# shiwanghua/swh-trl

Measured on AMD Instinct MI355X. Metric: GRPO step samples/sec (rollout+update), Qwen2.5-0.5B at 1/2/4/8 MI355X, higher is better.
Workload: dtype bf16; 1 GPU; configs[1]: Qwen2.5-0.5B GRPO bf16, group_size=8, 256-tok completions; model=Qwen2.5-0.5B (random init), global_batch=64, prompts_per_gpu=8, prompt_len=128, completion_len=256, seq_len=384, micro_batch=16, grad_accum=4, parallelism=dp1, layers=24

## Files before the change

include/swh_trl_amd.h:

```cpp
#ifndef SWH_TRL_AMD_H
#define SWH_TRL_AMD_H

#include <stdint.h>

#ifdef __cplusplus
extern "C" {
#endif

#define SWH_OK 0
#define SWH_E_ARG (-1)
#define SWH_E_LAUNCH (-2)
#define SWH_E_DTYPE (-3)

#define SWH_F32 0
#define SWH_BF16 1
#define SWH_F16 2

const char *swh_version(void);
const char *swh_status_string(int status);

typedef struct swh_launch_policy {
    int64_t wide_kmin;
    int32_t wide_gemm;
    int32_t wide_smax;
    int32_t wide_cb;
    int32_t gemm_ms;
    int32_t gemm_cb;
    int32_t gemm_s;
    int32_t gemm_persist;
    int32_t gemm_wn;
    int32_t gemm_tile;
    int32_t gemm_nw;
    int32_t xstream;
    int32_t lm_ring14;
    int32_t filt_wgs;
    int32_t wide_waves;
    int32_t attn_pair;
} swh_launch_policy;
int swh_launch_policy_default(swh_launch_policy *out);
int swh_get_launch_policy(swh_launch_policy *out);
int swh_set_launch_policy(const swh_launch_policy *p);

#define SWH_LOGP_ROUND_SCALED 1
int swh_logp_entropy_fwd(const void *logits, int dtype, int64_t rows_outer, int64_t rows_inner,
                         int64_t stride_outer, int64_t stride_inner, int64_t V, const int64_t *ids,
                         float temperature, int flags, float *logp, float *entropy, float *lse,
                         void *stream);

int swh_logp_bwd(const void *logits, int dtype, int64_t rows_outer, int64_t rows_inner,
                 int64_t stride_outer, int64_t stride_inner, int64_t V, const int64_t *ids,
                 float temperature, int flags, const float *lse, const float *dlogp, void *dlogits,
                 int64_t dstride_outer, int64_t dstride_inner, void *stream);
int swh_log_softmax_gather_exact(const void *logits, int dtype, int64_t rows_outer, int64_t rows_inner,
                                 int64_t stride_outer, int64_t stride_inner, int64_t V, const int64_t *ids,
                                 void *out, void *stream);


typedef struct {
    float temperature;
    float top_p;
    float min_p;
    float repetition_penalty;
    int32_t top_k;
    int32_t greedy;
    int32_t min_new_tokens;
    int32_t pad_token_id;
    int32_t n_eos;
    int32_t eos_ids[4];
} swh_sample_params;
int64_t swh_sample_workspace_bytes(int64_t B, int64_t V);
int swh_sample_step(const void *logits, int dtype, int64_t B, int64_t V, int64_t ld,
                    const swh_sample_params *params, const uint64_t *rng, const int32_t *step,
                    int32_t *finished,
                    uint32_t *seen, int64_t *out_tokens, int64_t out_ld, int64_t *cur_tokens,
                    float *out_logp, float *scores_out, void *workspace, void *stream);
int swh_seen_init(const int64_t *ids, const int32_t *mask, int64_t B, int64_t L, int64_t V,
                  uint32_t *seen, void *stream);
int swh_step_advance(int32_t *step, void *stream);

int swh_completion_mask(const int64_t *completion_ids, int64_t B, int64_t C, const int32_t *eos_ids,
                        int32_t n_eos, int32_t mask_truncated, int32_t *mask, int32_t *lengths,
                        int32_t *has_eos, void *stream);

int swh_group_advantage(const float *rewards_per_func, const float *weights, int64_t N, int64_t F,
                        int64_t G, int32_t scale_rewards, float *advantages, float *rewards,
                        float *group_mean, float *group_std, int32_t *zero_std, void *stream);

#define SWH_LOSS_GRPO 0
#define SWH_LOSS_BNPO 1
#define SWH_LOSS_DR_GRPO 2
// ... 186 lines not shown
```

swh_trl_amd/_lib.py:

```python
from __future__ import annotations

import ctypes as C
import os
import threading

_HERE = os.path.dirname(os.path.abspath(__file__))
LIB_PATH = os.path.join(_HERE, "libswh_trl_amd.so")

c_i32, c_i64, c_f32, c_vp, c_u64 = C.c_int32, C.c_int64, C.c_float, C.c_void_p, C.c_uint64

SWH_F32, SWH_BF16, SWH_F16 = 0, 1, 2
SWH_LOGP_ROUND_SCALED = 1
LOSS_TYPES = {"grpo": 0, "bnpo": 1, "dr_grpo": 2}
IS_LEVELS = {"token": 0, "sequence": 1}


class AttnView(C.Structure):
    _fields_ = [("base", C.c_void_p * 2), ("sb", c_i64 * 2), ("sh", c_i64 * 2), ("sl", c_i64 * 2),
                ("div", c_i32 * 2)]


class SampleParams(C.Structure):
    _fields_ = [("temperature", c_f32), ("top_p", c_f32), ("min_p", c_f32), ("repetition_penalty", c_f32),
                ("top_k", c_i32), ("greedy", c_i32), ("min_new_tokens", c_i32), ("pad_token_id", c_i32),
                ("n_eos", c_i32), ("eos_ids", c_i32 * 4)]


class GRPOLossParams(C.Structure):
    _fields_ = [("beta", c_f32), ("epsilon_low", c_f32), ("epsilon_high", c_f32), ("delta", c_f32),
                ("loss_type", c_i32), ("is_level", c_i32), ("max_completion_length", c_i32),
                ("num_segments", c_i32)]


class LaunchPolicy(C.Structure):
    _fields_ = [("wide_kmin", c_i64), ("wide_gemm", c_i32), ("wide_smax", c_i32), ("wide_cb", c_i32),
                ("gemm_ms", c_i32), ("gemm_cb", c_i32), ("gemm_s", c_i32), ("gemm_persist", c_i32),
                ("gemm_wn", c_i32), ("gemm_tile", c_i32), ("gemm_nw", c_i32), ("xstream", c_i32),
                ("lm_ring14", c_i32), ("filt_wgs", c_i32), ("wide_waves", c_i32), ("attn_pair", c_i32)]


SIGNATURES = {
    "swh_version": (C.c_char_p, []),
    "swh_status_string": (C.c_char_p, [c_i32]),
    "swh_launch_policy_default": (c_i32, [C.POINTER(LaunchPolicy)]),
    "swh_get_launch_policy": (c_i32, [C.POINTER(LaunchPolicy)]),
    "swh_set_launch_policy": (c_i32, [C.POINTER(LaunchPolicy)]),
    "swh_logp_entropy_fwd": (c_i32, [c_vp, c_i32, c_i64, c_i64, c_i64, c_i64, c_i64, c_vp, c_f32, c_i32,
                                     c_vp, c_vp, c_vp, c_vp]),
    "swh_log_softmax_gather_exact": (c_i32, [c_vp, c_i32, c_i64, c_i64, c_i64, c_i64, c_i64, c_vp, c_vp, c_vp]),
    "swh_logp_bwd": (c_i32, [c_vp, c_i32, c_i64, c_i64, c_i64, c_i64, c_i64, c_vp, c_f32, c_i32, c_vp, c_vp,
                             c_vp, c_i64, c_i64, c_vp]),
    "swh_sample_workspace_bytes": (c_i64, [c_i64, c_i64]),
    "swh_sample_step": (c_i32, [c_vp, c_i32, c_i64, c_i64, c_i64, C.POINTER(SampleParams), c_vp, c_vp, c_vp,
                                c_vp, c_vp, c_i64, c_vp, c_vp, c_vp, c_vp, c_vp]),
    "swh_seen_init": (c_i32, [c_vp, c_vp, c_i64, c_i64, c_i64, c_vp, c_vp]),
    "swh_step_advance": (c_i32, [c_vp, c_vp]),
    "swh_completion_mask": (c_i32, [c_vp, c_i64, c_i64, c_vp, c_i32, c_i32, c_vp, c_vp, c_vp, c_vp]),
    "swh_group_advantage": (c_i32, [c_vp, c_vp, c_i64, c_i64, c_i64, c_i32, c_vp, c_vp, c_vp, c_vp, c_vp,
                                    c_vp]),
    "swh_grpo_loss_workspace_bytes": (c_i64, [c_i64]),
    "swh_grpo_loss_fwd_bwd": (c_i32, [c_vp, c_vp, c_vp, c_vp, c_vp, c_vp, c_vp, c_vp, c_vp, c_i64, c_i64,
                                      C.POINTER(GRPOLossParams), c_vp, c_vp, c_vp, c_vp, c_vp, c_vp]),
    "swh_masked_whiten_workspace_bytes": (c_i64, [c_i64]),
    "swh_masked_whiten": (c_i32, [c_vp, c_vp, c_i64, c_i32, c_vp, c_vp, c_vp, c_vp]),
    "swh_gae_scan": (c_i32, [c_vp, c_vp, c_i64, c_i64, c_f32, c_f32, c_vp, c_vp, c_vp]),
    "swh_ppo_loss_workspace_bytes": (c_i64, [c_i64]),
    "swh_ppo_loss_fwd_bwd": (c_i32, [c_vp, c_vp, c_vp, c_vp, c_vp, c_vp, c_vp, c_vp, c_i64, c_i64, c_f32,
                                     c_f32, c_f32, c_vp, c_vp, c_vp, c_vp, c_vp, c_vp]),
    "swh_ppo_truncate": (c_i32, [c_vp, c_i64, c_i64, c_i64, c_i64, c_vp, c_vp, c_vp]),
    "swh_ppo_rewards": (c_i32, [c_vp, c_vp, c_i64, c_i64, c_i64, c_f32, c_i32, c_f32, c_i32, c_vp, c_vp, c_vp, c_vp,
                                c_i32, c_vp, c_vp, c_vp, c_vp, c_vp, c_vp]),
    "swh_value_head_fwd": (c_i32, [c_vp, c_i32, c_i64, c_i64, c_i64, c_vp, c_vp, c_vp, c_vp]),
    "swh_sqnorm_partials": (c_i64, [c_i64]),
    "swh_grad_sqnorm": (c_i32, [c_vp, c_i32, c_i64, c_vp, c_vp]),
    "swh_finalize_clip": (c_i32, [c_vp, c_i64, c_f32, c_vp, c_vp]),
    "swh_adamw": (c_i32, [c_vp, c_vp, c_vp, c_vp, c_i32, c_vp, c_i32, c_i64, c_f32, c_f32, c_f32, c_f32, c_f32,
                          c_i64, c_vp, c_vp, c_i32, c_vp]),
    "swh_accumulate": (c_i32, [c_vp, c_vp, c_i32, c_i64, c_f32, c_vp]),
    "swh_dw_reduce": (c_i32, [c_vp, c_i32, c_i64, c_vp, c_i32, c_vp]),
    "swh_gemm_nt": (c_i32, [c_vp, c_vp, c_vp, c_vp, c_i64, c_i64, c_i64, c_i64, c_i64, c_i64, c_vp]),
    "swh_gemm_nt256": (c_i32, [c_vp, c_vp, c_vp, c_vp, c_i64, c_i64, c_i64, c_i64, c_i64, c_i64, c_vp]),
    "swh_gemm_tn_partials": (c_i32, [c_vp, c_vp, c_vp, c_vp, c_i64, c_i64, c_i64, c_i64, c_i64, c_i32, c_vp]),
    "swh_gemm_tn256_partials": (c_i32, [c_vp, c_vp, c_vp, c_i64, c_i64, c_i64, c_i64, c_i64, c_i32, c_vp]),
    "swh_gemm_tn_fold": (c_i32, [c_vp, c_i32, c_i64, c_vp, c_i32, c_vp]),
    "swh_ema_mix": (c_i32, [c_vp, c_vp, c_i32, c_i64, c_f32, c_f32, c_vp]),
    "swh_rmsnorm_fwd": (c_i32, [c_vp, c_vp, c_vp, c_vp, c_i64, c_i64, c_f32, c_vp, c_vp, c_i32, c_vp]),
    "swh_rmsnorm_bwd": (c_i32, [c_vp, c_vp, c_vp, c_vp, c_i64, c_i64, c_vp, c_vp, c_i64, c_vp, c_i32, c_vp]),
    "swh_rmsnorm_dw_accum": (c_i32, [c_vp, c_i64, c_i64, c_vp, c_i32, c_vp]),
    "swh_colsum_partials": (c_i32, [c_vp, c_i64, c_i64, c_i64, c_vp, c_i32, c_vp]),
    "swh_layernorm_fwd": (c_i32, [c_vp, c_vp, c_vp, c_vp, c_i64, c_i64, c_f32, c_vp, c_vp, c_vp, c_vp, c_i32, c_vp]),
    "swh_layernorm_bwd_partial_rows": (c_i64, [c_i64, c_i64]),
# ... 153 lines not shown
```

swh_trl_amd/csrc/decode.hip:

```cpp
#include <cstdio>
#include <cstdlib>
#include <type_traits>

#include "common.hpp"

namespace swh {
int wide_gemm(const void *x, const void *w, int64_t M, int64_t N, int64_t K, float eps, const float *ss_in,
              const void *bias, void *residual, int32_t silu, void *y, int64_t ldy, float *ss_out, void *workspace,
              int64_t workspace_bytes, int64_t counter_bytes, int32_t packed, hipStream_t stream);
int64_t wide_gemm_slab_bytes(int64_t M, int64_t N, int64_t K, int32_t silu);
bool wide_gemm_eligible(int64_t M, int64_t N, int64_t K, int32_t silu);
int wide_pack(const void *src, const void *norm_w, int64_t N, int64_t K, int32_t silu, void *dst, hipStream_t stream);
int wide_lm_sample(const void *x, const void *w, int64_t M, int64_t V, int64_t K, float eps, const float *ss_in,
                   const swh_sample_params &p, const uint64_t *rng, const int32_t *step, LmPart *part, int *pstride,
                   hipStream_t stream);
int frag_pack(const void *src, const void *norm_w, int64_t N, int64_t K, int32_t silu, void *dst, hipStream_t stream);

namespace {

typedef __bf16 bf16x8 __attribute__((ext_vector_type(8)));
typedef float f32x4 __attribute__((ext_vector_type(4)));

constexpr int kRows = 64;
constexpr int64_t kCounterBytes = 1 << 16;

enum : int { EPI_PLAIN = 0, EPI_RESIDUAL = 1, EPI_SILU = 2 };

#ifdef SWH_GEMM_TRACE_ON
__device__ unsigned long long *g_gemm_trace;
#define SWH_GEMM_TRACE(i)                                                                                      \
    if (threadIdx.x == 0 && g_gemm_trace)                                                                      \
    g_gemm_trace[((int64_t)(blockIdx.z * gridDim.y + blockIdx.y) * gridDim.x + blockIdx.x) * 8 + (i)] =        \
        wall_clock64()
#else
#define SWH_GEMM_TRACE(i)
#endif

__device__ __forceinline__ void lds_barrier() { asm volatile("s_waitcnt lgkmcnt(0)\n\ts_barrier" ::: "memory"); }

__device__ __forceinline__ bf16x8 as_bf16x8(const uint4 &v) { return __builtin_bit_cast(bf16x8, v); }

typedef float f32x2 __attribute__((ext_vector_type(2)));
typedef __bf16 bf16x2 __attribute__((ext_vector_type(2)));
__device__ __forceinline__ uint32_t norm_pair(uint32_t xv, f32x2 w, float rs) {
    const f32x2 xf = {__uint_as_float(xv << 16), __uint_as_float(xv & 0xffff0000u)};
    const uint32_t tb = __builtin_bit_cast(uint32_t, __builtin_convertvector(xf * rs, bf16x2));
    const f32x2 tf = {__uint_as_float(tb << 16), __uint_as_float(tb & 0xffff0000u)};
    return __builtin_bit_cast(uint32_t, __builtin_convertvector(tf * w, bf16x2));
}
__device__ __forceinline__ uint4 norm_frag(const uint4 &xv, const float4 &w0, const float4 &w1, float rs) {
    return uint4{norm_pair(xv.x, f32x2{w0.x, w0.y}, rs), norm_pair(xv.y, f32x2{w0.z, w0.w}, rs),
                 norm_pair(xv.z, f32x2{w1.x, w1.y}, rs), norm_pair(xv.w, f32x2{w1.z, w1.w}, rs)};
}

__device__ __forceinline__ uint4 pack8(const float *v) {
    uint32_t o[4];
#pragma unroll
    for (int k = 0; k < 4; ++k)
        o[k] = (uint32_t)f32_to_bf16_bits(v[2 * k]) | ((uint32_t)f32_to_bf16_bits(v[2 * k + 1]) << 16);
    return uint4{o[0], o[1], o[2], o[3]};
}


struct GemmLds {
    int64_t nw_off, ss_off, body_off, xs_bytes, slots_off, total;
};
__host__ __device__ inline GemmLds gemm_lds(int cb, int mr, int nw, int krmax, int K, int nm, bool persist,
                                            int wn = 1) {
    GemmLds L;
    L.nw_off = 512;
    L.ss_off = L.nw_off + (nm == 1 ? (int64_t)krmax * 4 : 0);
    L.body_off = L.ss_off + (nm ? ((int64_t)mr * (K / 64) * 4 + 15) / 16 * 16 : 0);
    L.xs_bytes = (int64_t)mr * (krmax * 2 + 16);
    const int wk = nw / wn;
    const int64_t slots = (int64_t)(wk + 1) * 16 * cb * (mr + 4) * 4;
    L.slots_off = L.body_off + (persist ? L.xs_bytes : 0);
    int64_t end = L.body_off + L.xs_bytes;
    if (L.slots_off + slots > end) end = L.slots_off + slots;
    L.total = end;
    return L;
}


#ifndef SWH_KU
#define SWH_KU 4
#endif
#ifndef SWH_ROUND_PREFETCH
#define SWH_ROUND_PREFETCH 0
#endif
#ifndef SWH_W_NT
#define SWH_W_NT 0
#endif
__device__ __forceinline__ uint4 ld_w(const uint16_t *p) {
// ... 558 lines not shown
                    float b[8];
                    unpack16<SWH_BF16>(pre_ep, b);
#pragma unroll
                    for (int cc = 0; cc < 8; ++cc) v[cc] += b[cc];
                }
                *reinterpret_cast<uint4 *>(y + (int64_t)gr * ldy + gc) = pack8(v);
            }
        }
    }
    if constexpr (EPI == EPI_RESIDUAL) {
        if (ss_out) {
            __syncthreads();
            if (tid < MR && m0 + tid < M) {
                float ss = 0.f;
#pragma unroll
                for (int cc = 0; cc < 16; ++cc) ss = fmaf(slot(F, tid, cc), slot(F, tid, cc), ss);
                ss_out[(int64_t)(m0 + tid) * (N / 16) + n0 / 16] = ss;
            }
        }
    }
    SWH_GEMM_TRACE(6);
}

constexpr int kLmMaxKS = 32;

struct LmSample {
    swh_sample_params p;
    const uint64_t *rng;
    const int32_t *step;
    LmPart *part;
    int pstride;
    int fw = 0;
    int yf = 0;
    float2 *lpart = nullptr;
};

template <int CTRL>
__device__ __forceinline__ float dpp_f(float v) {
    return __builtin_bit_cast(float, __builtin_amdgcn_update_dpp(0, __builtin_bit_cast(int, v), CTRL, 0xF, 0xF, false));
}
__device__ __forceinline__ float row16_max(float v) {
    v = fmaxf(v, dpp_f<0xB1>(v));
    v = fmaxf(v, dpp_f<0x4E>(v));
    v = fmaxf(v, dpp_f<0x141>(v));
    return fmaxf(v, dpp_f<0x140>(v));
}
__device__ __forceinline__ float row16_sum(float v) {
    v += dpp_f<0xB1>(v);
    v += dpp_f<0x4E>(v);
    v += dpp_f<0x141>(v);
    return v + dpp_f<0x140>(v);
}

template <int NM, int EPI, bool BIAS, int SAMPLE, int KSC, int RD = 0>
__global__ __launch_bounds__(RD ? 768 : 512) void lm_head_kernel(const uint16_t *__restrict__ x, const uint16_t *__restrict__ w,
                                                      int M, int N, int K, const uint16_t *__restrict__ norm_w,
                                                      float eps, const float *__restrict__ ss_in,
                                                      const uint16_t *__restrict__ bias, uint16_t *__restrict__ y,
                                                      int ldy, LmSample smp) {
    extern __shared__ __attribute__((aligned(16))) unsigned char lds[];
    const int tid = threadIdx.x, lane = tid & 63, wid = tid >> 6, NT = blockDim.x, NW = NT >> 6;
    const int rl = lane & 15, kq = (lane >> 4) * 8, g = lane >> 4;
    const int nmt = (M + 63) / 64, mt = blockIdx.x % nmt, m0 = mt * 64;
    const int wgs = gridDim.x / nmt, wg = blockIdx.x / nmt;
    constexpr int KSA = KSC ? KSC : kLmMaxKS;
    const int ntile = (EPI == EPI_SILU) ? N / 8 : N / 16, KS = KSC ? KSC : K / 32, RS = K * 2 + 16;
    const GemmLds L = gemm_lds(1, 64, NW, K, K, NM, false);
    float *rstd_s = reinterpret_cast<float *>(lds);
    float *nw_s = reinterpret_cast<float *>(lds + L.nw_off);
    float *ssp = reinterpret_cast<float *>(lds + L.ss_off);
    unsigned char *xs = lds + L.body_off;
    const int tstep = wgs * NW;
    int t = wg + wgs * wid;
    SWH_GEMM_TRACE(0);

    static_assert(RD == 0 || (KSC != 0 && KSC % RD == 0 && 2 * RD == KSC), "RD: half of a compile-time tile");
    constexpr int KR = RD ? RD : KSA;
    uint4 bv[KR];
    auto wrow_of = [&](int tile) -> int64_t {
        if constexpr (EPI == EPI_SILU) return (rl < 8) ? tile * 8 + rl : N + tile * 8 + rl - 8;
        return (int64_t)tile * 16 + rl;
    };
    const int64_t wst = smp.fw ? 512 : 32;
    auto wbase = [&](int tile) -> const uint16_t * {
        return smp.fw ? w + ((int64_t)tile * KS * 64 + lane) * 8 : w + wrow_of(tile) * K + kq;
    };
    auto issue = [&](int tile) {
        const uint16_t *wr = wbase(tile);
#pragma unroll
        for (int ks = 0; ks < KR; ++ks)
            if (KSC || ks < KS) bv[ks] = ld_wt<EPI == EPI_SILU>(wr + ks * wst);
    };
    if (t < ntile) issue(t);
    const int nc = K / 64;
    const bool reg_rstd = NM == 2 && ss_in && 64 * 8 <= NT && nc <= 64;
    const bool use_ss = NM && ss_in && 64 * nc <= 4 * NT && !reg_rstd;
    float4 ssv[4];
    float4 ss8[8];
    uint4 nwv[2];
    if (reg_rstd) {
        const int r = min(m0 + (tid >> 3), M - 1), sub = tid & 7;
        const float4 *row = reinterpret_cast<const float4 *>(ss_in + (int64_t)r * (K / 16));
#pragma unroll
        for (int j = 0; j < 8; ++j)
            if (sub + 8 * j < nc) ss8[j] = row[sub + 8 * j];
    }
    if constexpr (NM != 0) {
        if (use_ss) {
#pragma unroll
            for (int q = 0; q < 4; ++q) {
                const int idx = min(tid + q * NT, 64 * nc - 1);
                const int r = idx / nc, c = idx - r * nc;
                ssv[q] = reinterpret_cast<const float4 *>(ss_in + (int64_t)min(m0 + r, M - 1) * (K / 16))[c];
            }
        }
        if constexpr (NM == 1) {
#pragma unroll
            for (int q = 0; q < 2; ++q) nwv[q] = reinterpret_cast<const uint4 *>(norm_w)[min(tid + q * NT, K / 8 - 1)];
        }
    }
    const int ppr = K / 8, jpl = (ppr + 63) >> 6;
    for (int r = wid; r < 64; r += NW) {
        const uint16_t *src = x + (int64_t)min(m0 + r, M - 1) * K;
        for (int j = 0; j < jpl; ++j) {
            const int c = lane + 64 * j;
            if (c < ppr)
                __builtin_amdgcn_global_load_lds(src + c * 8,
                                                 (__attribute__((address_space(3))) void *)(xs + r * RS + j * 1024),
                                                 16, 0, 0);
        }
    }
    if constexpr (NM != 0) {
        if (use_ss) {
#pragma unroll
            for (int q = 0; q < 4; ++q) {
                const int idx = tid + q * NT;
                if (idx < 64 * nc) ssp[idx] = ((ssv[q].x + ssv[q].y) + ssv[q].z) + ssv[q].w;
            }
        }
#pragma unroll
        for (int q = 0; q < 2; ++q)
            if (NM == 1 && tid + q * NT < K / 8) {
                float f[8];
                unpack16<SWH_BF16>(nwv[q], f);
                reinterpret_cast<float4 *>(nw_s)[2 * (tid + q * NT)] = float4{f[0], f[1], f[2], f[3]};
                reinterpret_cast<float4 *>(nw_s)[2 * (tid + q * NT) + 1] = float4{f[4], f[5], f[6], f[7]};
            }
    }
    SWH_GEMM_TRACE(1);
    asm volatile("s_waitcnt vmcnt(0)" ::: "memory");
    if (reg_rstd) {
        const int r = tid >> 3, sub = tid & 7;
        float v = 0.f;
#pragma unroll
        for (int j = 0; j < 8; ++j)
            if (sub + 8 * j < nc) v += ((ss8[j].x + ss8[j].y) + ss8[j].z) + ss8[j].w;
        v += __shfl_xor(v, 1);
        v += __shfl_xor(v, 2);
        v += __shfl_xor(v, 4);
        if (r < 64 && sub == 0) rstd_s[r] = rsqrtf(v / (float)K + eps);
    }
    lds_barrier();
    SWH_GEMM_TRACE(2);
    if (NM != 0 && !reg_rstd) {
        if (tid < 64) {
            float ssum = 0.f;
            if (use_ss) {
                for (int c = 0; c < nc; ++c) ssum += ssp[tid * nc + c];
            } else {
                for (int c = 0; c < ppr; ++c) {
                    float a[8];
                    unpack16<SWH_BF16>(*reinterpret_cast<const uint4 *>(xs + tid * RS + c * 16), a);
#pragma unroll
                    for (int k = 0; k < 8; ++k) ssum = fmaf(a[k], a[k], ssum);
                }
            }
            rstd_s[tid] = rsqrtf(ssum / (float)K + eps);
        }
        lds_barrier();
    }
    SWH_GEMM_TRACE(3);
    float rsr[4][4];
#pragma unroll
    for (int i = 0; i < 4; ++i)
#pragma unroll
        for (int e = 0; e < 4; ++e) rsr[i][e] = (NM == 2) ? rstd_s[i * 16 + 4 * g + e] : 1.f;
    if constexpr (NM == 1) {
        int r = tid / ppr, c = tid - r * ppr;
        const int rstep = NT / ppr, cstep = NT - rstep * ppr;
        while (r < 64) {
            uint4 *pv = reinterpret_cast<uint4 *>(xs + r * RS + c * 16);
            const float4 *wv = reinterpret_cast<const float4 *>(nw_s) + 2 * c;
            *pv = norm_frag(*pv, wv[0], wv[1], rstd_s[r]);
            r += rstep;
            c += cstep;
            if (c >= ppr) {
                c -= ppr;
                ++r;
            }
        }
        lds_barrier();
    }
    constexpr bool TDIV = SAMPLE == 2 || SAMPLE == 4, LOGP = SAMPLE >= 3;
    float bk[4][4];
    int32_t bi[4][4];
    uint32_t k0 = 0, k1 = 0, clo = 0, chi = 0;
    bool suppress = false;
    float temp = 1.f;
    float lm_run = kNegInf, ls_run = 0.f;
    if constexpr (SAMPLE) {
#pragma unroll
        for (int i = 0; i < 4; ++i)
#pragma unroll
            for (int e = 0; e < 4; ++e) {
                bk[i][e] = kNegInf;
                bi[i][e] = 0x7fffffff;
            }
        const int32_t step = *smp.step;
        const uint64_t seed = smp.rng[0], ctr = smp.rng[1] + (uint64_t)step;
        k0 = (uint32_t)seed;
        k1 = (uint32_t)(seed >> 32);
        clo = (uint32_t)ctr;
        chi = (uint32_t)(ctr >> 32);
        suppress = step < smp.p.min_new_tokens;
        temp = (!smp.p.greedy && smp.p.temperature != 1.0f) ? smp.p.temperature : 1.f;
    }
    for (; t < ntile; t += tstep) {
        f32x4 acc[4];
#pragma unroll
        for (int i = 0; i < 4; ++i) acc[i] = f32x4{0.f, 0.f, 0.f, 0.f};
        const unsigned char *xrow = xs + rl * RS + kq * 2;
        const bool ring = SWH_LM_RING && KSC != 0 && t + tstep < ntile;
        const uint16_t *wnext = wbase(ring ? t + tstep : t);
        const uint16_t *wcur = wbase(t);
        if constexpr (KSC != 0) {
            constexpr int APF = 1, AR = APF + 1;
            uint4 a[AR][4];
#pragma unroll
            for (int p = 0; p < APF; ++p)
#pragma unroll
                for (int i = 0; i < 4; ++i) a[p][i] = *reinterpret_cast<const uint4 *>(xrow + i * 16 * RS + p * 64);
#pragma unroll
            for (int ks = 0; ks < KSC; ++ks) {
                if (ks + APF < KSC) {
#pragma unroll
                    for (int i = 0; i < 4; ++i)
                        a[(ks + APF) % AR][i] = *reinterpret_cast<const uint4 *>(xrow + i * 16 * RS + (ks + APF) * 64);
                }
#pragma unroll
                for (int i = 0; i < 4; ++i)
                    acc[i] = __builtin_amdgcn_mfma_f32_16x16x32_bf16(as_bf16x8(a[ks % AR][i]), as_bf16x8(bv[ks % KR]),
                                                                    acc[i], 0, 0, 0);
                if constexpr (RD != 0) {
                    if (ks + KR < KSC) bv[ks % KR] = ld_wt<EPI == EPI_SILU>(wcur + (ks + KR) * wst);
                    else if (ring) bv[ks % KR] = ld_wt<EPI == EPI_SILU>(wnext + (ks + KR - KSC) * wst);
                } else if (ring) {
                    bv[ks] = ld_wt<EPI == EPI_SILU>(wnext + ks * wst);
                }
                __builtin_amdgcn_sched_barrier(0);
            }
        } else {
#pragma unroll
            for (int ks = 0; ks < KSA; ++ks) {
                if (ks < KS) {
#pragma unroll
                    for (int i = 0; i < 4; ++i) {
                        const uint4 a = *reinterpret_cast<const uint4 *>(xrow + i * 16 * RS + ks * 64);
                        acc[i] = __builtin_amdgcn_mfma_f32_16x16x32_bf16(as_bf16x8(a), as_bf16x8(bv[ks]), acc[i], 0, 0, 0);
                    }
                }
            }
        }
        if (!ring && t + tstep < ntile) issue(t + tstep);
        SWH_GEMM_TRACE(4);
        if constexpr (SAMPLE) {
            const int col = t * 16 + rl;
            float mask_add = 0.f;
            if (suppress) {
#pragma unroll
                for (int e = 0; e < 4; ++e)
                    if (e < smp.p.n_eos && col == smp.p.eos_ids[e]) mask_add = kNegInf;
            }
            float own_m = kNegInf, own_s = 0.f;
#pragma unroll
            for (int i = 0; i < 4; ++i) {
                U4 rw{0u, 0u, 0u, 0u};
                if (!smp.p.greedy) rw = philox4x32_10(U4{(uint32_t)col, (uint32_t)((m0 >> 2) + 4 * i + g), clo, chi}, k0, k1);
                const uint32_t wd[4] = {rw.x, rw.y, rw.z, rw.w};
// ... 932 lines not shown
    return launch_xstream_kw<8, MS, NM, EPI, BIAS>(c, s, X, W, m, n, k, eps, ss_in, Bs, R, ss_out, Y, ld);
}

int launch_xstream(const GemmCfg &c, hipStream_t s, const uint16_t *X, const uint16_t *W, int m, int n, int k, int nm,
                   float eps, const float *ss_in, const uint16_t *Bs, uint16_t *R, float *ss_out, uint16_t *Y, int ld) {
    const bool lds_image = !launch_policy().xstream;
    const int ks = k / 32;
    if ((lds_image && !c.xf) || c.cb != 1 || c.wn != 1 || c.s != 1 || c.persist || c.nw != 8 || n % 16 ||
        ks < 8 || ks > (c.xf ? 152 : 64) || (c.ms != 1 && c.ms != 2))
        return 1;
    if (R) {
        if (nm != 0 || Bs || c.ms != 1) return 1;
        if (c.xf) {
            if (m % 16 || (ks + 7) / 8 > 19) return 1;
            if ((ks + 7) / 8 > 8)
                return launch_xstream_kw<19, 1, 0, EPI_RESIDUAL, false>(c, s, X, W, m, n, k, eps, nullptr, nullptr, R,
                                                                       ss_out, nullptr, ld);
        }
        return launch_xstream_ms<1, 0, EPI_RESIDUAL, false>(c, s, X, W, m, n, k, eps, nullptr, nullptr, R, ss_out, nullptr,
                                                            ld);
    }
    if (c.xf) return 1;
    if (nm != 2 || !ss_in || !Bs || !Y) return 1;
    if (c.ms == 1)
        return launch_xstream_ms<1, 2, EPI_PLAIN, true>(c, s, X, W, m, n, k, eps, ss_in, Bs, nullptr, nullptr, Y, ld);
    return launch_xstream_ms<2, 2, EPI_PLAIN, true>(c, s, X, W, m, n, k, eps, ss_in, Bs, nullptr, nullptr, Y, ld);
}

template <int MS, int NM, int EPI, bool BIAS>
int launch_gemm_cb(const GemmCfg &c, dim3 grid, size_t lds, hipStream_t s, const uint16_t *X, const uint16_t *W,
                   int m, int n, int k, const uint16_t *NWt, float eps, const float *ss_in, const uint16_t *Bs,
                   uint16_t *R, float *ss_out, uint16_t *Y, int ld, float *slab, int *ctr) {
    switch (c.cb / c.wn) {
    case 1:
        if (c.nw > 8)
            return launch_gemm<1, MS, NM, EPI, BIAS, 1024>(c, grid, lds, s, X, W, m, n, k, NWt, eps, ss_in, Bs, R, ss_out, Y, ld, slab, ctr);
        return launch_gemm<1, MS, NM, EPI, BIAS, 512>(c, grid, lds, s, X, W, m, n, k, NWt, eps, ss_in, Bs, R, ss_out, Y, ld, slab, ctr);
    case 2: return launch_gemm<2, MS, NM, EPI, BIAS, 512>(c, grid, lds, s, X, W, m, n, k, NWt, eps, ss_in, Bs, R, ss_out, Y, ld, slab, ctr);
    default: return launch_gemm<4, MS, NM, EPI, BIAS, 512>(c, grid, lds, s, X, W, m, n, k, NWt, eps, ss_in, Bs, R, ss_out, Y, ld, slab, ctr);
    }
}

template <int NM, int EPI, bool BIAS>
int launch_gemm_ms(const GemmCfg &c, dim3 grid, size_t lds, hipStream_t s, const uint16_t *X, const uint16_t *W,
                   int m, int n, int k, const uint16_t *NWt, float eps, const float *ss_in, const uint16_t *Bs,
                   uint16_t *R, float *ss_out, uint16_t *Y, int ld, float *slab, int *ctr) {
    switch (c.ms) {
    case 1: return launch_gemm_cb<1, NM, EPI, BIAS>(c, grid, lds, s, X, W, m, n, k, NWt, eps, ss_in, Bs, R, ss_out, Y, ld, slab, ctr);
    case 2: return launch_gemm_cb<2, NM, EPI, BIAS>(c, grid, lds, s, X, W, m, n, k, NWt, eps, ss_in, Bs, R, ss_out, Y, ld, slab, ctr);
    default: return launch_gemm_cb<4, NM, EPI, BIAS>(c, grid, lds, s, X, W, m, n, k, NWt, eps, ss_in, Bs, R, ss_out, Y, ld, slab, ctr);
    }
}

template <int NM, int EPI, bool BIAS, int SAMPLE, int KSC, int RD = 0>
int launch_lm_ks(dim3 grid, size_t lds, hipStream_t s, const uint16_t *X, const uint16_t *W, int M, int N, int K,
                 const uint16_t *NWt, float eps, const float *ss_in, const uint16_t *Bs, uint16_t *Y, int ldy,
                 const LmSample &smp) {
    if (!lds_opt_in<&lm_head_kernel<NM, EPI, BIAS, SAMPLE, KSC, RD>>()) return SWH_E_LAUNCH;
    lm_head_kernel<NM, EPI, BIAS, SAMPLE, KSC, RD><<<grid, RD ? 768 : 512, lds, s>>>(X, W, M, N, K, NWt, eps, ss_in, Bs,
                                                                                  Y, ldy, smp);
    return launch_status();
}

inline bool lm_ring14() { return launch_policy().lm_ring14 != 0; }

template <int NM, int EPI, bool BIAS, int SAMPLE>
int launch_lm(dim3 grid, size_t lds, hipStream_t s, const uint16_t *X, const uint16_t *W, int M, int N, int K,
              const uint16_t *NWt, float eps, const float *ss_in, const uint16_t *Bs, uint16_t *Y, int ldy,
              const LmSample &smp) {
    if constexpr (SAMPLE == 1 || SAMPLE == 3) {
        if (!smp.p.greedy && smp.p.temperature != 1.0f)
            return launch_lm<NM, EPI, BIAS, SAMPLE + 1>(grid, lds, s, X, W, M, N, K, NWt, eps, ss_in, Bs, Y, ldy, smp);
    }
    switch (K / 32) {
    case 28:
        if ((SAMPLE == 1 || SAMPLE == 2) && lm_ring14())
            return launch_lm_ks<NM, EPI, BIAS, SAMPLE, 28, 14>(grid, lds, s, X, W, M, N, K, NWt, eps, ss_in, Bs, Y, ldy,
                                                               smp);
        return launch_lm_ks<NM, EPI, BIAS, SAMPLE, 28>(grid, lds, s, X, W, M, N, K, NWt, eps, ss_in, Bs, Y, ldy, smp);
    case 32: return launch_lm_ks<NM, EPI, BIAS, SAMPLE, 32>(grid, lds, s, X, W, M, N, K, NWt, eps, ss_in, Bs, Y, ldy, smp);
    default: return launch_lm_ks<NM, EPI, BIAS, SAMPLE, 0>(grid, lds, s, X, W, M, N, K, NWt, eps, ss_in, Bs, Y, ldy, smp);
    }
}


template <int EPI, bool BIAS>
int launch_tiles(int nm, dim3 grid, size_t lds, hipStream_t s, const uint16_t *X, const uint16_t *W, int M, int N,
                 int K, const uint16_t *NWt, float eps, const float *ss_in, const uint16_t *Bs, uint16_t *Y, int ldy,
                 int fw, int yf = 0) {
    LmSample none{};
    none.fw = fw;
    none.yf = yf;
    if (nm == 1) return launch_lm<1, EPI, BIAS, false>(grid, lds, s, X, W, M, N, K, NWt, eps, ss_in, Bs, Y, ldy, none);
    if (nm == 2) return launch_lm<2, EPI, BIAS, false>(grid, lds, s, X, W, M, N, K, nullptr, eps, ss_in, Bs, Y, ldy, none);
    return launch_lm<0, EPI, BIAS, false>(grid, lds, s, X, W, M, N, K, nullptr, eps, nullptr, Bs, Y, ldy, none);
}

}
}

using namespace swh;

static int attn_decode_impl(const void *qkv, void *k_cache, void *v_cache, const float *rope_cos,
                            const float *rope_sin, const int32_t *prompt_len, const int32_t *prompt_row,
                            const int32_t *state, int64_t B, int32_t Hq, int32_t Hkv, int32_t D, int32_t Tmax,
                            float scale, void *out, int32_t out_frag, AttnPrefetch pf, void *stream) {
    if (!qkv || !k_cache || !v_cache || !rope_cos || !rope_sin || !prompt_len || !state || !out || B < 0 || Hkv <= 0 ||
        Hq % Hkv || Tmax <= 0 || B > 65535 || (out_frag & ~1))
        return SWH_E_ARG;
    if (out_frag && (B % 16 || (Hq * D) % 32 || (reinterpret_cast<uintptr_t>(out) & 15))) return SWH_E_ARG;
    if (B == 0) return SWH_OK;
    hipStream_t s = static_cast<hipStream_t>(stream);
    const auto *q = static_cast<const uint16_t *>(qkv);
    auto *kc = static_cast<uint16_t *>(k_cache), *vc = static_cast<uint16_t *>(v_cache);
    auto *o = static_cast<uint16_t *>(out);
    const int gq = Hq / Hkv;
    pf.rows = (int)B;
    pf.prow = prompt_row;
    pf.ofrag = out_frag;
    if (D == 64) return attn_dispatch_gq<64>(gq, q, kc, vc, rope_cos, rope_sin, prompt_len, state, B, Hq, Hkv, Tmax, scale, o, s, pf);
    if (D == 128) return attn_dispatch_gq<128>(gq, q, kc, vc, rope_cos, rope_sin, prompt_len, state, B, Hq, Hkv, Tmax, scale, o, s, pf);
    return SWH_E_ARG;
}

extern "C" int swh_attn_decode_shared_frag(const void *qkv, void *k_cache, void *v_cache, const float *rope_cos,
                                           const float *rope_sin, const int32_t *prompt_len,
                                           const int32_t *prompt_row, const int32_t *state, int64_t B, int32_t Hq,
                                           int32_t Hkv, int32_t D, int32_t Tmax, float scale, void *out,
                                           int32_t out_frag, void *stream) {
    return attn_decode_impl(qkv, k_cache, v_cache, rope_cos, rope_sin, prompt_len, prompt_row, state, B, Hq, Hkv, D,
                            Tmax, scale, out, out_frag, AttnPrefetch{}, stream);
}
extern "C" int swh_attn_decode_l3(const void *qkv, void *k_cache, void *v_cache, const float *rope_cos,
// ... 342 lines not shown
```

swh_trl_amd/csrc/lib.hip:

```cpp
#include "common.hpp"

namespace swh {

int cu_count() {
    int dev = 0;
    if (hipGetDevice(&dev) != hipSuccess || dev < 0 || dev >= kMaxDevices) return 256;
    static std::once_flag once[kMaxDevices];
    static int cus[kMaxDevices];
    std::call_once(once[dev], [dev] {
        int n = 0;
        cus[dev] = hipDeviceGetAttribute(&n, hipDeviceAttributeMultiprocessorCount, dev) == hipSuccess && n > 0 ? n : 256;
    });
    return cus[dev];
}

bool lds_opt_in_once(const void *kernel, std::once_flag *once, bool *ok) {
    int dev = 0;
    if (hipGetDevice(&dev) != hipSuccess || dev < 0 || dev >= kMaxDevices) return false;
    std::call_once(once[dev], [&] {
        ok[dev] = hipFuncSetAttribute(kernel, hipFuncAttributeMaxDynamicSharedMemorySize, kMaxDynLds) == hipSuccess;
    });
    return ok[dev];
}

namespace {
swh_launch_policy default_policy() {
    swh_launch_policy p{};
    p.wide_kmin = 2048;
    p.wide_gemm = 1;
    p.wide_smax = 8;
    p.xstream = 1;
    p.lm_ring14 = 1;
    p.filt_wgs = 1024;
    p.attn_pair = 1;
    return p;
}
thread_local swh_launch_policy t_policy = default_policy();

bool in(int32_t v, std::initializer_list<int32_t> ok) {
    for (int32_t o : ok)
        if (v == o) return true;
    return false;
}
}

swh_launch_policy launch_policy() { return t_policy; }

}

using namespace swh;

extern "C" int swh_launch_policy_default(swh_launch_policy *out) {
    if (!out) return SWH_E_ARG;
    *out = default_policy();
    return SWH_OK;
}

extern "C" int swh_get_launch_policy(swh_launch_policy *out) {
    if (!out) return SWH_E_ARG;
    *out = launch_policy();
    return SWH_OK;
}

extern "C" int swh_set_launch_policy(const swh_launch_policy *p) {
    if (!p) return SWH_E_ARG;
    const bool geo_auto = p->gemm_ms == 0;
    if (p->wide_kmin < 32 || !in(p->wide_gemm, {0, 1}) || p->wide_smax < 1 || p->wide_smax > 8 ||
        !in(p->wide_cb, {0, 1, 2}) || !in(p->gemm_ms, {0, 1, 2, 4}) ||
        (geo_auto ? (p->gemm_cb || p->gemm_s || p->gemm_persist || p->gemm_wn)
                  : (!in(p->gemm_cb, {1, 2, 4}) || p->gemm_s < 1 || p->gemm_s > 8 || !in(p->gemm_persist, {0, 1}) ||
                     !in(p->gemm_wn, {1, 2, 4}))) ||
        !in(p->gemm_tile, {0, 1}) || !in(p->gemm_nw, {0, 4, 8, 16}) || !in(p->xstream, {0, 1}) ||
        !in(p->lm_ring14, {0, 1}) || p->filt_wgs < 64 || p->filt_wgs > 65536 || !in(p->wide_waves, {0, 6, 7, 8}) ||
        !in(p->attn_pair, {0, 1}))
        return SWH_E_ARG;
    t_policy = *p;
    return SWH_OK;
}

extern "C" const char *swh_version(void) { return "swh_trl_amd 0.1.0 (gfx950)"; }

extern "C" const char *swh_status_string(int status) {
    switch (status) {
    case SWH_OK: return "ok";
    case SWH_E_ARG: return "invalid argument";
    case SWH_E_LAUNCH: return "kernel launch failed";
    case SWH_E_DTYPE: return "unsupported dtype";
    default: return "unknown status";
    }
}
```

Before: 200.6 samples/s.

## Pipeline first-tile weight loads with split activation DMA in lm_head prologue

Adds a PIPE variant of the lm_head/decode GEMM kernel for compile-time K of 896 or 1024 with no sampling. The first tile's weight loads are interleaved with two asynchronous global-to-LDS DMA halves of the activation block, and MFMA work on the first half of K starts before the second half has landed. The RMS-norm rstd is computed from precomputed sum-of-squares after the first tile. This targets the serialized prologue (load activations, wait, barrier, then load weights) in small-M decode GEMMs. It adds a new template instantiation, inline asm waitcnt accounting that must match the load counts exactly, and a policy knob that is on by default.

```diff
diff --git a/include/swh_trl_amd.h b/include/swh_trl_amd.h
--- a/include/swh_trl_amd.h
+++ b/include/swh_trl_amd.h
@@ -36,6 +36,7 @@
     int32_t filt_wgs;
     int32_t wide_waves;
     int32_t attn_pair;
+    int32_t tile_pipe;
 } swh_launch_policy;
 int swh_launch_policy_default(swh_launch_policy *out);
 int swh_get_launch_policy(swh_launch_policy *out);
diff --git a/swh_trl_amd/_lib.py b/swh_trl_amd/_lib.py
--- a/swh_trl_amd/_lib.py
+++ b/swh_trl_amd/_lib.py
@@ -36,7 +36,8 @@
     _fields_ = [("wide_kmin", c_i64), ("wide_gemm", c_i32), ("wide_smax", c_i32), ("wide_cb", c_i32),
                 ("gemm_ms", c_i32), ("gemm_cb", c_i32), ("gemm_s", c_i32), ("gemm_persist", c_i32),
                 ("gemm_wn", c_i32), ("gemm_tile", c_i32), ("gemm_nw", c_i32), ("xstream", c_i32),
-                ("lm_ring14", c_i32), ("filt_wgs", c_i32), ("wide_waves", c_i32), ("attn_pair", c_i32)]
+                ("lm_ring14", c_i32), ("filt_wgs", c_i32), ("wide_waves", c_i32), ("attn_pair", c_i32),
+                ("tile_pipe", c_i32)]
 
 
 SIGNATURES = {
diff --git a/swh_trl_amd/csrc/decode.hip b/swh_trl_amd/csrc/decode.hip
--- a/swh_trl_amd/csrc/decode.hip
+++ b/swh_trl_amd/csrc/decode.hip
@@ -39,6 +39,34 @@
 __device__ __forceinline__ void lds_barrier() { asm volatile("s_waitcnt lgkmcnt(0)\n\ts_barrier" ::: "memory"); }
 
 __device__ __forceinline__ bf16x8 as_bf16x8(const uint4 &v) { return __builtin_bit_cast(bf16x8, v); }
+
+__device__ __forceinline__ bf16x8 as_bf16x8(const u32x4 &v) { return __builtin_bit_cast(bf16x8, v); }
+template <bool NT>
+__device__ __forceinline__ void ldw_hidden(u32x4 &d, const uint16_t *p) {
+    if constexpr (NT) asm volatile("global_load_dwordx4 %0, %1, off nt" : "=v"(d) : "v"(p) : "memory");
+    else asm volatile("global_load_dwordx4 %0, %1, off" : "=v"(d) : "v"(p) : "memory");
+}
+template <int OFF>
+__device__ __forceinline__ void lds128_hidden(u32x4 &d, uint32_t base) {
+    static_assert(OFF >= 0 && OFF < 65536, "ds_read offset field");
+    asm volatile("ds_read_b128 %0, %1 offset:%2" : "=v"(d) : "v"(base), "n"(OFF) : "memory");
+}
+template <int N>
+__device__ __forceinline__ void vm_wait() {
+    asm volatile("s_waitcnt vmcnt(%0)" ::"n"(N) : "memory");
+}
+__device__ __forceinline__ void landed(u32x4 &d) { asm volatile("" : "+v"(d)); }
+template <int N>
+__device__ __forceinline__ void lgkm_wait(u32x4 (&a)[4]) {
+    asm volatile("s_waitcnt lgkmcnt(%4)" : "+v"(a[0]), "+v"(a[1]), "+v"(a[2]), "+v"(a[3]) : "n"(N) : "memory");
+}
+template <int I, int N, class F>
+__device__ __forceinline__ void static_for(F &&f) {
+    if constexpr (I < N) {
+        f(std::integral_constant<int, I>{});
+        static_for<I + 1, N>(f);
+    }
+}
 
 typedef float f32x2 __attribute__((ext_vector_type(2)));
 typedef __bf16 bf16x2 __attribute__((ext_vector_type(2)));
@@ -703,7 +731,7 @@
     return v + dpp_f<0x140>(v);
 }
 
-template <int NM, int EPI, bool BIAS, int SAMPLE, int KSC, int RD = 0>
+template <int NM, int EPI, bool BIAS, int SAMPLE, int KSC, int RD = 0, int PIPE = 0>
 __global__ __launch_bounds__(RD ? 768 : 512) void lm_head_kernel(const uint16_t *__restrict__ x, const uint16_t *__restrict__ w,
                                                       int M, int N, int K, const uint16_t *__restrict__ norm_w,
                                                       float eps, const float *__restrict__ ss_in,
@@ -742,10 +770,10 @@
         for (int ks = 0; ks < KR; ++ks)
             if (KSC || ks < KS) bv[ks] = ld_wt<EPI == EPI_SILU>(wr + ks * wst);
     };
-    if (t < ntile) issue(t);
+    if (PIPE == 0 && t < ntile) issue(t);
     const int nc = K / 64;
-    const bool reg_rstd = NM == 2 && ss_in && 64 * 8 <= NT && nc <= 64;
-    const bool use_ss = NM && ss_in && 64 * nc <= 4 * NT && !reg_rstd;
+    const bool reg_rstd = PIPE == 0 && NM == 2 && ss_in && 64 * 8 <= NT && nc <= 64;
+    const bool use_ss = PIPE == 0 && NM && ss_in && 64 * nc <= 4 * NT && !reg_rstd;
     float4 ssv[4];
     float4 ss8[8];
     uint4 nwv[2];
@@ -771,7 +799,7 @@
         }
     }
     const int ppr = K / 8, jpl = (ppr + 63) >> 6;
-    for (int r = wid; r < 64; r += NW) {
+    for (int r = PIPE ? 64 : wid; r < 64; r += NW) {
         const uint16_t *src = x + (int64_t)min(m0 + r, M - 1) * K;
         for (int j = 0; j < jpl; ++j) {
             const int c = lane + 64 * j;
@@ -798,8 +826,10 @@
                 reinterpret_cast<float4 *>(nw_s)[2 * (tid + q * NT) + 1] = float4{f[4], f[5], f[6], f[7]};
             }
     }
-    SWH_GEMM_TRACE(1);
-    asm volatile("s_waitcnt vmcnt(0)" ::: "memory");
+    if constexpr (PIPE == 0) {
+        SWH_GEMM_TRACE(1);
+        asm volatile("s_waitcnt vmcnt(0)" ::: "memory");
+    }
     if (reg_rstd) {
         const int r = tid >> 3, sub = tid & 7;
         float v = 0.f;
@@ -811,9 +841,11 @@
         v += __shfl_xor(v, 4);
         if (r < 64 && sub == 0) rstd_s[r] = rsqrtf(v / (float)K + eps);
     }
-    lds_barrier();
-    SWH_GEMM_TRACE(2);
-    if (NM != 0 && !reg_rstd) {
+    if constexpr (PIPE == 0) {
+        lds_barrier();
+        SWH_GEMM_TRACE(2);
+    }
+    if (PIPE == 0 && NM != 0 && !reg_rstd) {
         if (tid < 64) {
             float ssum = 0.f;
             if (use_ss) {
@@ -829,6 +861,100 @@
             rstd_s[tid] = rsqrtf(ssum / (float)K + eps);
         }
         lds_barrier();
+    }
+    f32x4 acc[4];
+    bool piped = false;
+    if constexpr (PIPE != 0) {
+        static_assert(KSC > 16 && KSC <= 32 && RD == 0 && NM != 1 && SAMPLE == 0,
+                      "the pipelined prologue: compile-time K of two DMA runs per row, 8 waves, no image pass");
+        constexpr int KS0 = 16, KC = KSC * 32, RSC = KC * 2 + 16, PPR = KC / 8, NCC = KC / 64;
+        constexpr int NSS = NM == 2 ? 2 : 0;
+        const bool own = __builtin_amdgcn_readfirstlane(t < ntile ? 1 : 0) != 0;
+        const uint16_t *wr = wbase(own ? t : 0);
+        u32x4 wv[KSC];
+        auto dma = [&](int j) __attribute__((always_inline)) {
+#pragma unroll
+            for (int q = 0; q < 8; ++q) {
+                const int r = wid + 8 * q, c = lane + 64 * j;
+                const uint16_t *src = x + (int64_t)min(m0 + r, M - 1) * KC;
+                if (c < PPR)
+                    __builtin_amdgcn_global_load_lds(src + c * 8,
+                                                     (__attribute__((address_space(3))) void *)(xs + r * RSC + j * 1024),
+                                                     16, 0, 0);
+            }
+        };
+        if (own) static_for<0, KS0>([&](auto k) __attribute__((always_inline)) {
+            ldw_hidden<EPI == EPI_SILU>(wv[decltype(k)::value], wr + decltype(k)::value * wst);
+        });
+        __builtin_amdgcn_sched_barrier(0);
+        dma(0);
+        __builtin_amdgcn_sched_barrier(0);
+        if (own) static_for<KS0, KSC>([&](auto k) __attribute__((always_inline)) {
+            ldw_hidden<EPI == EPI_SILU>(wv[decltype(k)::value], wr + decltype(k)::value * wst);
+        });
+        __builtin_amdgcn_sched_barrier(0);
+        dma(1);
+        __builtin_amdgcn_sched_barrier(0);
+        float4 st[2];
+        if constexpr (NM == 2) {
+            const float4 *row =
+                reinterpret_cast<const float4 *>(ss_in + (int64_t)min(m0 + (tid >> 3), M - 1) * (KC / 16));
+            st[0] = row[tid & 7];
+            st[1] = row[min((tid & 7) + 8, NCC - 1)];
+        }
+        __builtin_amdgcn_sched_barrier(0);
+        SWH_GEMM_TRACE(1);
+        if (own) vm_wait<KSC - KS0 + 8 + NSS>();
+        else vm_wait<8 + NSS>();
+        lds_barrier();
+        SWH_GEMM_TRACE(7);
+#pragma unroll
+        for (int i = 0; i < 4; ++i) acc[i] = f32x4{0.f, 0.f, 0.f, 0.f};
+        const uint32_t xa0 = (uint32_t)(uintptr_t)(const __attribute__((address_space(3))) unsigned char *)(
+            xs + rl * RSC + kq * 2);
+        const uint32_t xa2 = xa0 + 32 * RSC;
+        u32x4 a[2][4];
+        auto read_a = [&](auto k, u32x4(&d)[4]) __attribute__((always_inline)) {
+            constexpr int ks = decltype(k)::value;
+            lds128_hidden<ks * 64>(d[0], xa0);
+            lds128_hidden<16 * RSC + ks * 64>(d[1], xa0);
+            lds128_hidden<ks * 64>(d[2], xa2);
+            lds128_hidden<16 * RSC + ks * 64>(d[3], xa2);
+        };
+        auto mma_chunk = [&](auto k0, auto k1) __attribute__((always_inline)) {
+            constexpr int K0 = decltype(k0)::value, K1 = decltype(k1)::value;
+            static_for<K0, K1>([&](auto k) __attribute__((always_inline)) { landed(wv[decltype(k)::value]); });
+            read_a(k0, a[K0 & 1]);
+            static_for<K0, K1>([&](auto k) __attribute__((always_inline)) {
+                constexpr int ks = decltype(k)::value;
+                if constexpr (ks + 1 < K1) read_a(std::integral_constant<int, ks + 1>{}, a[(ks + 1) & 1]);
+                lgkm_wait<(ks + 1 < K1) ? 4 : 0>(a[ks & 1]);
+                __builtin_amdgcn_sched_barrier(0);
+#pragma unroll
+                for (int i = 0; i < 4; ++i)
+                    acc[i] = __builtin_amdgcn_mfma_f32_16x16x32_bf16(as_bf16x8(a[ks & 1][i]), as_bf16x8(wv[ks]), acc[i],
+                                                                    0, 0, 0);
+                __builtin_amdgcn_sched_barrier(0);
+            });
+        };
+        if (own) mma_chunk(std::integral_constant<int, 0>{}, std::integral_constant<int, KS0>{});
+        vm_wait<0>();
+        lds_barrier();
+        SWH_GEMM_TRACE(2);
+        if (own) mma_chunk(std::integral_constant<int, KS0>{}, std::integral_constant<int, KSC>{});
+        piped = own;
+        if constexpr (NM == 2) {
+            const int r = tid >> 3, sub = tid & 7;
+            float v = 0.f;
+#pragma unroll
+            for (int j = 0; j < 2; ++j)
+                if (sub + 8 * j < NCC) v += ((st[j].x + st[j].y) + st[j].z) + st[j].w;
+            v += __shfl_xor(v, 1);
+            v += __shfl_xor(v, 2);
+            v += __shfl_xor(v, 4);
+            if (sub == 0) rstd_s[r] = rsqrtf(v / (float)KC + eps);
+            lds_barrier();
+        }
     }
     SWH_GEMM_TRACE(3);
     float rsr[4][4];
@@ -877,14 +1003,18 @@
         temp = (!smp.p.greedy && smp.p.temperature != 1.0f) ? smp.p.temperature : 1.f;
     }
     for (; t < ntile; t += tstep) {
-        f32x4 acc[4];
-#pragma unroll
-        for (int i = 0; i < 4; ++i) acc[i] = f32x4{0.f, 0.f, 0.f, 0.f};
+        const bool mma = !(PIPE != 0 && piped);
+        piped = false;
+        if (mma) {
+#pragma unroll
+            for (int i = 0; i < 4; ++i) acc[i] = f32x4{0.f, 0.f, 0.f, 0.f};
+        }
         const unsigned char *xrow = xs + rl * RS + kq * 2;
-        const bool ring = SWH_LM_RING && KSC != 0 && t + tstep < ntile;
+        const bool ring = mma && SWH_LM_RING && KSC != 0 && t + tstep < ntile;
         const uint16_t *wnext = wbase(ring ? t + tstep : t);
         const uint16_t *wcur = wbase(t);
-        if constexpr (KSC != 0) {
+        if (!mma) {
+        } else if constexpr (KSC != 0) {
             constexpr int APF = 1, AR = APF + 1;
             uint4 a[AR][4];
 #pragma unroll
@@ -1923,17 +2053,22 @@
     }
 }
 
-template <int NM, int EPI, bool BIAS, int SAMPLE, int KSC, int RD = 0>
+template <int NM, int EPI, bool BIAS, int SAMPLE, int KSC, int RD = 0, int PIPE = 0>
 int launch_lm_ks(dim3 grid, size_t lds, hipStream_t s, const uint16_t *X, const uint16_t *W, int M, int N, int K,
                  const uint16_t *NWt, float eps, const float *ss_in, const uint16_t *Bs, uint16_t *Y, int ldy,
                  const LmSample &smp) {
-    if (!lds_opt_in<&lm_head_kernel<NM, EPI, BIAS, SAMPLE, KSC, RD>>()) return SWH_E_LAUNCH;
-    lm_head_kernel<NM, EPI, BIAS, SAMPLE, KSC, RD><<<grid, RD ? 768 : 512, lds, s>>>(X, W, M, N, K, NWt, eps, ss_in, Bs,
-                                                                                  Y, ldy, smp);
+    if (!lds_opt_in<&lm_head_kernel<NM, EPI, BIAS, SAMPLE, KSC, RD, PIPE>>()) return SWH_E_LAUNCH;
+    lm_head_kernel<NM, EPI, BIAS, SAMPLE, KSC, RD, PIPE><<<grid, RD ? 768 : 512, lds, s>>>(X, W, M, N, K, NWt, eps, ss_in,
+                                                                                        Bs, Y, ldy, smp);
     return launch_status();
 }
 
 inline bool lm_ring14() { return launch_policy().lm_ring14 != 0; }
+
+template <int NM, int SAMPLE>
+inline bool tile_pipe(const float *ss_in) {
+    return SAMPLE == 0 && (NM == 0 || (NM == 2 && ss_in)) && launch_policy().tile_pipe != 0;
+}
 
 template <int NM, int EPI, bool BIAS, int SAMPLE>
 int launch_lm(dim3 grid, size_t lds, hipStream_t s, const uint16_t *X, const uint16_t *W, int M, int N, int K,
@@ -1948,8 +2083,19 @@
         if ((SAMPLE == 1 || SAMPLE == 2) && lm_ring14())
             return launch_lm_ks<NM, EPI, BIAS, SAMPLE, 28, 14>(grid, lds, s, X, W, M, N, K, NWt, eps, ss_in, Bs, Y, ldy,
                                                                smp);
+        if constexpr (SAMPLE == 0 && NM != 1) {
+            if (tile_pipe<NM, SAMPLE>(ss_in))
+                return launch_lm_ks<NM, EPI, BIAS, SAMPLE, 28, 0, 1>(grid, lds, s, X, W, M, N, K, NWt, eps, ss_in, Bs, Y,
+                                                                    ldy, smp);
+        }
         return launch_lm_ks<NM, EPI, BIAS, SAMPLE, 28>(grid, lds, s, X, W, M, N, K, NWt, eps, ss_in, Bs, Y, ldy, smp);
-    case 32: return launch_lm_ks<NM, EPI, BIAS, SAMPLE, 32>(grid, lds, s, X, W, M, N, K, NWt, eps, ss_in, Bs, Y, ldy, smp);
+    case 32:
+        if constexpr (SAMPLE == 0 && NM != 1) {
+            if (tile_pipe<NM, SAMPLE>(ss_in))
+                return launch_lm_ks<NM, EPI, BIAS, SAMPLE, 32, 0, 1>(grid, lds, s, X, W, M, N, K, NWt, eps, ss_in, Bs, Y,
+                                                                    ldy, smp);
+        }
+        return launch_lm_ks<NM, EPI, BIAS, SAMPLE, 32>(grid, lds, s, X, W, M, N, K, NWt, eps, ss_in, Bs, Y, ldy, smp);
     default: return launch_lm_ks<NM, EPI, BIAS, SAMPLE, 0>(grid, lds, s, X, W, M, N, K, NWt, eps, ss_in, Bs, Y, ldy, smp);
     }
 }
diff --git a/swh_trl_amd/csrc/lib.hip b/swh_trl_amd/csrc/lib.hip
--- a/swh_trl_amd/csrc/lib.hip
+++ b/swh_trl_amd/csrc/lib.hip
@@ -33,6 +33,7 @@
     p.lm_ring14 = 1;
     p.filt_wgs = 1024;
     p.attn_pair = 1;
+    p.tile_pipe = 1;
     return p;
 }
 thread_local swh_launch_policy t_policy = default_policy();
@@ -72,7 +73,7 @@
                      !in(p->gemm_wn, {1, 2, 4}))) ||
         !in(p->gemm_tile, {0, 1}) || !in(p->gemm_nw, {0, 4, 8, 16}) || !in(p->xstream, {0, 1}) ||
         !in(p->lm_ring14, {0, 1}) || p->filt_wgs < 64 || p->filt_wgs > 65536 || !in(p->wide_waves, {0, 6, 7, 8}) ||
-        !in(p->attn_pair, {0, 1}))
+        !in(p->attn_pair, {0, 1}) || !in(p->tile_pipe, {0, 1}))
         return SWH_E_ARG;
     t_policy = *p;
     return SWH_OK;
```

New measurement: 203.4 samples/s (median of 6 runs). 1.4% higher.
